# GeeeG/CloudAAE

Measured on AMD Instinct MI355X. Metric: point-clouds/sec (train step, N=1024), higher is better.
Workload: dtype f32, the dgcnn_agg products as error-free 3 x bf16 splits on the bf16 matrix cores (fp32 accumulate); 1 GPU; CloudAAE train step: get_model_dgcnn_mean_6d, all 21 YCB classes, batch 32/GPU, N=1024 points, k=10, 4N-point Chamfer target, TF-Adam; global_batch=32, per_gpu_batch=32, num_point=1024, parallelism=dp1, step_issue=recorded step replay

## Files before the change

cloudaae_amd/csrc/gemm_x3.hip:

```cpp
#include "common.h"
#include "gemm.h"
#include "bn_common.h"
#include "../../include/cloudaae_hip.h"

namespace cloudaae {

typedef float f32x16 __attribute__((ext_vector_type(16)));
typedef __bf16 bf16x8 __attribute__((ext_vector_type(8)));
typedef __bf16 bf16x2 __attribute__((ext_vector_type(2)));
typedef unsigned int u32x4v __attribute__((ext_vector_type(4)));

constexpr int X3_BK = 32;
constexpr int X3_LDK = 40;
constexpr int X3_THREADS = 256;

enum { X3_STORE = 0, X3_ACCUM = 1, X3_ATOMIC = 2 };

constexpr float X3_H_MAX = __builtin_bit_cast(float, 0x7f7f7fffu);
__device__ __forceinline__ void split3(float v, __bf16 &h, __bf16 &m, __bf16 &l)
{
    h = (__bf16)__builtin_amdgcn_fmed3f(v, -X3_H_MAX, X3_H_MAX);
    const float r1 = v - (float)h;
    m = (__bf16)r1;
    l = (__bf16)(r1 - (float)m);
}
__device__ __forceinline__ unsigned pack_pair(__bf16 lo, __bf16 hi)
{
    const bf16x2 p = {lo, hi};
    unsigned w;
    __builtin_memcpy(&w, &p, 4);
    return w;
}

template <int ROWS, bool KC>
struct Slab3 {
    static constexpr int ITEMS = KC ? ROWS * (X3_BK / 4) : (X3_BK / 2) * (ROWS / 4);
    static constexpr int PER = (ITEMS + X3_THREADS - 1) / X3_THREADS;
    static constexpr int PLANE = ROWS * X3_LDK;
    float4v r0[2][PER], r1[2][KC ? 1 : PER];
    unsigned boff[PER];
    static_assert(ROWS % 32 == 0, "tile sides are multiples of 32");
    static __device__ __forceinline__ int item_kp(int it) { return ((it >> 5) & 3) * 4 + (it & 3); }
    static __device__ __forceinline__ int item_oq(int it) { return (it >> 7) * 8 + ((it >> 2) & 7); }
    static __device__ __forceinline__ bool live(int it) { return ITEMS % X3_THREADS == 0 || it < ITEMS; }

    __device__ __forceinline__ void init(int ld)
    {
#pragma unroll
        for (int u = 0; u < PER; ++u) {
            const int it = u * X3_THREADS + (int)threadIdx.x;
            if (KC)
                boff[u] = 4u * (unsigned)((it / (X3_BK / 4)) * ld + 4 * (it % (X3_BK / 4)));
            else
                boff[u] = 4u * (unsigned)(2 * item_kp(it) * ld + 4 * item_oq(it));
        }
    }
    template <int SET>
    __device__ __forceinline__ void load(const float *__restrict__ P0, int ld)
    {
        const char *base = reinterpret_cast<const char *>(P0);
        const char *base1 = reinterpret_cast<const char *>(P0 + ld);
#pragma unroll
        for (int u = 0; u < PER; ++u) {
            const int it = u * X3_THREADS + (int)threadIdx.x;
            if (live(it)) {
                r0[SET][u] = *reinterpret_cast<const float4v *>(base + boff[u]);
                if (!KC)
                    r1[SET][u] = *reinterpret_cast<const float4v *>(base1 + boff[u]);
            }
        }
    }
    template <int SET>
    __device__ __forceinline__ void stage(__bf16 *__restrict__ lds) const
    {
#pragma unroll
        for (int u = 0; u < PER; ++u) {
            const int it = u * X3_THREADS + (int)threadIdx.x;
            if (!live(it))
                continue;
            __bf16 a[3][4];
            split3(r0[SET][u].x, a[0][0], a[1][0], a[2][0]);
            split3(r0[SET][u].y, a[0][1], a[1][1], a[2][1]);
            split3(r0[SET][u].z, a[0][2], a[1][2], a[2][2]);
            split3(r0[SET][u].w, a[0][3], a[1][3], a[2][3]);
            if (KC) {
                const int o = it / (X3_BK / 4), kq = it % (X3_BK / 4);
#pragma unroll
                for (int p = 0; p < 3; ++p) {
                    const unsigned w0 = pack_pair(a[p][0], a[p][1]), w1 = pack_pair(a[p][2], a[p][3]);
                    const uint2 w = {w0, w1};
                    *reinterpret_cast<uint2 *>(lds + p * PLANE + o * X3_LDK + 4 * kq) = w;
                }
            } else {
                __bf16 b[3][4];
                split3(r1[SET][u].x, b[0][0], b[1][0], b[2][0]);
                split3(r1[SET][u].y, b[0][1], b[1][1], b[2][1]);
                split3(r1[SET][u].z, b[0][2], b[1][2], b[2][2]);
                split3(r1[SET][u].w, b[0][3], b[1][3], b[2][3]);
                const int kp = item_kp(it), oq = item_oq(it);
                const int rot = (oq >> 1) & 3;
                const bool r1_ = (rot & 1) != 0, r2_ = (rot & 2) != 0;
#pragma unroll
                for (int p = 0; p < 3; ++p) {
                    const unsigned p0 = pack_pair(a[p][0], b[p][0]), p1 = pack_pair(a[p][1], b[p][1]),
                                   p2 = pack_pair(a[p][2], b[p][2]), p3 = pack_pair(a[p][3], b[p][3]);
                    const unsigned t0 = r1_ ? p1 : p0, t1 = r1_ ? p2 : p1, t2 = r1_ ? p3 : p2, t3 = r1_ ? p0 : p3;
                    const unsigned q0 = r2_ ? t2 : t0, q1 = r2_ ? t3 : t1, q2 = r2_ ? t0 : t2, q3 = r2_ ? t1 : t3;
                    __bf16 *dst = lds + p * PLANE + (4 * oq) * X3_LDK + 2 * kp;
                    *reinterpret_cast<unsigned *>(dst + ((0 + rot) & 3) * X3_LDK) = q0;
                    *reinterpret_cast<unsigned *>(dst + ((1 + rot) & 3) * X3_LDK) = q1;
                    *reinterpret_cast<unsigned *>(dst + ((2 + rot) & 3) * X3_LDK) = q2;
                    *reinterpret_cast<unsigned *>(dst + ((3 + rot) & 3) * X3_LDK) = q3;
                }
            }
        }
    }
};

template <int BM, int BN>
constexpr int x3_lds_bytes() { return 3 * (BM + BN) * X3_LDK * 2; }

template <int BM, int BN, int WM, int WN, bool TA, bool TB, int DEPTH>
__global__ __launch_bounds__(X3_THREADS, 2) void gemm_x3_kernel(int M, int N, int K, const float *__restrict__ A, int lda,
                                                             const float *__restrict__ B, int ldb, float *__restrict__ C,
                                                             int ldc, const float *__restrict__ bias, int epilogue,
                                                             int kchunk, double *__restrict__ colstats)
{
    static_assert(WM * WN * 64 == X3_THREADS, "4 waves");
    constexpr int TM = BM / WM / 32, TN = BN / WN / 32;
    typedef Slab3<BM, !TA> SA;
    typedef Slab3<BN, TB> SB;
    extern __shared__ __attribute__((aligned(16))) unsigned char x3_lds[];
    __bf16 *ldsA = reinterpret_cast<__bf16 *>(x3_lds);
    __bf16 *ldsB = ldsA + 3 * SA::PLANE;

    const int lane = threadIdx.x & 63, wave = threadIdx.x >> 6;
    const int wm = wave / WN, wn = wave % WN;
    const int tiles = gridDim.x * gridDim.y;
    int vid, slice;
    if (gridDim.z > 1 && (gridDim.z & 7) == 0) {
        const int lin = (blockIdx.z * gridDim.y + blockIdx.y) * gridDim.x + blockIdx.x;
        const int u = lin >> 3;
        slice = (lin & 7) + 8 * (u / tiles);
        vid = u % tiles;
    } else {
        vid = xcd_contiguous(blockIdx.y * gridDim.x + blockIdx.x, tiles);
        slice = blockIdx.z;
    }
    const int m0 = (vid / (int)gridDim.x) * BM, n0 = (vid % (int)gridDim.x) * BN;
    const int kbeg = slice * kchunk;
    const int kend = min(K, kbeg + kchunk);
    f32x16 acc[TM][TN];
#pragma unroll
    for (int i = 0; i < TM; ++i)
#pragma unroll
        for (int j = 0; j < TN; ++j)
#pragma unroll
            for (int r = 0; r < 16; ++r)
                acc[i][j][r] = 0.0f;

    const float *pa = A + (TA ? (size_t)kbeg * lda + m0 : (size_t)m0 * lda + kbeg);
    const float *pb = B + (TB ? (size_t)n0 * ldb + kbeg : (size_t)kbeg * ldb + n0);
    const size_t stepa = TA ? (size_t)X3_BK * lda : (size_t)X3_BK;
    const size_t stepb = TB ? (size_t)X3_BK : (size_t)X3_BK * ldb;
    SA sa;
    SB sb;
    sa.init(lda);
    sb.init(ldb);
    const int fr = lane & 31, fk = lane >> 5;
    auto multiply = [&]() {
#pragma unroll
        for (int s = 0; s < X3_BK / 16; ++s) {
            bf16x8 a[3][TM], b[3][TN];
#pragma unroll
            for (int p = 0; p < 3; ++p) {
#pragma unroll
                for (int i = 0; i < TM; ++i)
                    a[p][i] = *reinterpret_cast<const bf16x8 *>(ldsA + p * SA::PLANE + ((wm * TM + i) * 32 + fr) * X3_LDK +
                                                                16 * s + 8 * fk);
#pragma unroll
                for (int j = 0; j < TN; ++j)
                    b[p][j] = *reinterpret_cast<const bf16x8 *>(ldsB + p * SB::PLANE + ((wn * TN + j) * 32 + fr) * X3_LDK +
                                                                16 * s + 8 * fk);
            }
#pragma unroll
            for (int i = 0; i < TM; ++i)
#pragma unroll
                for (int j = 0; j < TN; ++j) {
                    acc[i][j] = __builtin_amdgcn_mfma_f32_32x32x16_bf16(a[2][i], b[0][j], acc[i][j], 0, 0, 0);
                    acc[i][j] = __builtin_amdgcn_mfma_f32_32x32x16_bf16(a[0][i], b[2][j], acc[i][j], 0, 0, 0);
                    acc[i][j] = __builtin_amdgcn_mfma_f32_32x32x16_bf16(a[1][i], b[1][j], acc[i][j], 0, 0, 0);
                    acc[i][j] = __builtin_amdgcn_mfma_f32_32x32x16_bf16(a[1][i], b[0][j], acc[i][j], 0, 0, 0);
                    acc[i][j] = __builtin_amdgcn_mfma_f32_32x32x16_bf16(a[0][i], b[1][j], acc[i][j], 0, 0, 0);
                    acc[i][j] = __builtin_amdgcn_mfma_f32_32x32x16_bf16(a[0][i], b[0][j], acc[i][j], 0, 0, 0);
                }
        }
    };
    if (DEPTH == 2) {
        const int nslab = (kend - kbeg) / X3_BK;
        auto slab_a = [&](int i) { return pa + (size_t)(i < nslab ? i : nslab - 1) * stepa; };
        auto slab_b = [&](int i) { return pb + (size_t)(i < nslab ? i : nslab - 1) * stepb; };
        sa.template load<0>(slab_a(0), lda);
        sb.template load<0>(slab_b(0), ldb);
        __builtin_amdgcn_sched_barrier(0);
        sa.template load<1>(slab_a(1), lda);
        sb.template load<1>(slab_b(1), ldb);
        __builtin_amdgcn_sched_barrier(0);
        for (int i = 0; i < nslab; i += 2) {
            __syncthreads();
            sa.template stage<0>(ldsA);
            sb.template stage<0>(ldsB);
            __syncthreads();
            sa.template load<0>(slab_a(i + 2), lda);
            sb.template load<0>(slab_b(i + 2), ldb);
            __builtin_amdgcn_sched_barrier(0);
            multiply();
            __builtin_amdgcn_sched_barrier(0);
            __syncthreads();
            sa.template stage<1>(ldsA);
            sb.template stage<1>(ldsB);
            __syncthreads();
            sa.template load<1>(slab_a(i + 3), lda);
            sb.template load<1>(slab_b(i + 3), ldb);
            __builtin_amdgcn_sched_barrier(0);
            multiply();
            __builtin_amdgcn_sched_barrier(0);
        }
    } else {
        sa.template load<0>(pa, lda);
        sb.template load<0>(pb, ldb);
        for (int k0 = kbeg; k0 < kend; k0 += X3_BK) {
            __syncthreads();
            sa.template stage<0>(ldsA);
            sb.template stage<0>(ldsB);
            __syncthreads();
            if (k0 + X3_BK < kend) {
                pa += stepa;
                pb += stepb;
                sa.template load<0>(pa, lda);
                sb.template load<0>(pb, ldb);
            }
            multiply();
        }
    }

    const bool add_bias = bias != nullptr && (epilogue != X3_ATOMIC || slice == 0);
    if (colstats != nullptr) {
        __syncthreads();
        double (*cs)[WM][BN] = reinterpret_cast<double (*)[WM][BN]>(x3_lds);
#pragma unroll
        for (int j = 0; j < TN; ++j) {
            const int cl = (wn * TN + j) * 32 + fr;
            const float bv = add_bias ? bias[n0 + cl] : 0.0f;
            double s1 = 0.0, s2 = 0.0;
#pragma unroll
            for (int i = 0; i < TM; ++i)
#pragma unroll
                for (int r = 0; r < 16; ++r) {
                    const double v = (double)(acc[i][j][r] + bv);
                    s1 += v;
                    s2 += v * v;
                }
            s1 += __shfl_xor(s1, 32, 64);
            s2 += __shfl_xor(s2, 32, 64);
            if (fk == 0) {
                cs[0][wm][cl] = s1;
                cs[1][wm][cl] = s2;
            }
        }
        __syncthreads();
        for (int t = threadIdx.x; t < 2 * BN; t += X3_THREADS) {
            const int which = t / BN, cl = t % BN;
            double v = cs[which][0][cl];
#pragma unroll
            for (int w = 1; w < WM; ++w)
                v += cs[which][w][cl];
            colstats[((size_t)(m0 / BM) * 2 + which) * N + n0 + cl] = v;
        }
    }
    float *c0 = C + (size_t)(m0 + wm * TM * 32 + 4 * fk) * ldc + (n0 + wn * TN * 32 + fr);
#pragma unroll
    for (int j = 0; j < TN; ++j) {
        const float bv = add_bias ? bias[n0 + (wn * TN + j) * 32 + fr] : 0.0f;
#pragma unroll
        for (int i = 0; i < TM; ++i) {
#pragma unroll
            for (int r = 0; r < 16; ++r) {
                float *dst = c0 + (size_t)(i * 32 + (r & 3) + 8 * (r >> 2)) * ldc + j * 32;
                const float v = acc[i][j][r] + bv;
                if (epilogue == X3_STORE)
                    *dst = v;
                else if (epilogue == X3_ACCUM)
                    *dst = *dst + v;
                else
                    atomicAdd(dst, v);
            }
        }
    }
}

static bool gemm_x3_plan(int ta, int tb, int M, int N, int K, int &BM, int &BN, int &splits)
{
    if (M <= 0 || N <= 0 || K <= 0 || K % X3_BK != 0 || (ta && tb))
        return false;
    BM = (ta && M % 160 == 0 && M % 128 != 0) ? 160 : 128;
    BN = (!ta && tb && N % 160 == 0 && N % 128 != 0) ? 160 : 128;
    if (M % BM != 0 || N % BN != 0)
        return false;
    const long long tiles = (long long)(M / BM) * (N / BN);
    splits = 1;
    if (tiles < 256 && K >= 256) {
        splits = (int)((tiles <= 4 ? 256 : 512) / tiles);
        const int max_splits = K / 128 > 0 ? K / 128 : 1;
        if (splits > max_splits)
            splits = max_splits;
        if (splits < 1)
            splits = 1;
        if (splits > 8)
            splits = splits / 8 * 8;
    }
    return true;
}

template <int BM, int BN, int WM, int WN, bool TA, bool TB, int DEPTH>
static int launch_x3(const char *name, dim3 grid, hipStream_t s, int M, int N, int K, const float *A, int lda, const float *B,
                     int ldb, float *C, int ldc, const float *bias, int epi, int kchunk, double *cs)
{
    constexpr int bytes = x3_lds_bytes<BM, BN>();
    constexpr auto kernel = &gemm_x3_kernel<BM, BN, WM, WN, TA, TB, DEPTH>;
    CLOUDAAE_CHECK_HIP(allow_dynamic_lds<kernel>(bytes, bytes), name);
    hipLaunchKernelGGL(kernel, grid, dim3(X3_THREADS), bytes, s, M, N, K, A, lda, B, ldb, C,
                       ldc, bias, epi, kchunk, cs);
    return 0;
}


__device__ __forceinline__ void split8(const float4v &x, const float4v &y, bf16x8 &h, bf16x8 &m, bf16x8 &l)
{
    const float v[8] = {x.x, x.y, x.z, x.w, y.x, y.y, y.z, y.w};
#pragma unroll
    for (int e = 0; e < 8; ++e) {
        const __bf16 hh = (__bf16)__builtin_amdgcn_fmed3f(v[e], -X3_H_MAX, X3_H_MAX);
        const float r1 = v[e] - (float)hh;
        const __bf16 mm = (__bf16)r1;
        h[e] = hh;
        m[e] = mm;
        l[e] = (__bf16)(r1 - (float)mm);
    }
}

__global__ __launch_bounds__(256) void x3_split_kernel(int rows0, int K0, int tr0, __bf16 *__restrict__ planes0, int rows1, int K1,
                                                       int tr1, __bf16 *__restrict__ planes1, const float *__restrict__ src, int ld)
{
    const bool second = blockIdx.y != 0;
    const int rows = second ? rows1 : rows0, K = second ? K1 : K0, transposed = second ? tr1 : tr0;
    __bf16 *__restrict__ planes = second ? planes1 : planes0;
    const int units = K >> 3;
    const long long t = (long long)blockIdx.x * 256 + threadIdx.x;
    if (t >= (long long)rows * units)
        return;
    int n, u;
    float4v x, y;
    if (transposed) {
        n = (int)(t % rows);
        u = (int)(t / rows);
        const float *s = src + (size_t)(8 * u) * ld + n;
        x = float4v{s[0], s[(size_t)ld], s[(size_t)2 * ld], s[(size_t)3 * ld]};
        y = float4v{s[(size_t)4 * ld], s[(size_t)5 * ld], s[(size_t)6 * ld], s[(size_t)7 * ld]};
    } else {
        u = (int)(t % units);
        n = (int)(t / units);
        const float4v *s = reinterpret_cast<const float4v *>(src + (size_t)n * ld + 8 * u);
        x = s[0];
        y = s[1];
    }
    bf16x8 h, m, l;
    split8(x, y, h, m, l);
    const int step = u >> 1, q = (u & 1) ^ ((n >> 3) & 1);
    __bf16 *d = planes + ((size_t)step * 3 * rows + n) * 16 + q * 8;
    *reinterpret_cast<bf16x8 *>(d) = h;
    *reinterpret_cast<bf16x8 *>(d + (size_t)rows * 16) = m;
    *reinterpret_cast<bf16x8 *>(d + (size_t)2 * rows * 16) = l;
}

template <int TM, int TN, int AS>
struct X3S {
    static constexpr int BM = 128 * TM, BN = 32 * TN;
    static constexpr int A_WAVE = 32 * TM * 128;
    static constexpr int A_STAGE = 4 * A_WAVE;
    static constexpr int A_BYTES = AS * A_STAGE;
    static constexpr int P_PLANE = BN * 32;
    static constexpr int P_STAGE = 3 * P_PLANE;
    static constexpr int P_PIECES = 3 * TN;
    static constexpr int LDS = A_BYTES + 3 * P_STAGE;
    static constexpr int JB = (TN - 1) / 2;
    static constexpr int T_STAGE = BN_DYC * 32 * 4;
    static constexpr int LDS_BNB = LDS + AS * T_STAGE;
};

struct X3BnBwd {
    const float *consts;
    float *dy;
    int lddy, rows, relu;
};

template <int TM, int TN, int AS, bool BNB>
__global__ __launch_bounds__(256, 2) void gemm_x3s_kernel(int M, int N, int K, const float *__restrict__ A, int lda,
                                                          const __bf16 *__restrict__ P, float *__restrict__ C, int ldc,
                                                          const float *__restrict__ bias, int accumulate,
                                                          double *__restrict__ colstats, X3BnBwd f)
{
    typedef X3S<TM, TN, AS> G;
    extern __shared__ __attribute__((aligned(16))) unsigned char x3_lds[];
    const int lane = threadIdx.x & 63;
    const int wave = __builtin_amdgcn_readfirstlane((int)(threadIdx.x >> 6));
    const int fr = lane & 31, fk = lane >> 5;
    const int tiles_n = N / G::BN;
    const int vid = xcd_contiguous(blockIdx.x, gridDim.x);
    const int m0 = (vid / tiles_n) * G::BM, n0 = (vid % tiles_n) * G::BN;
    const int nslab = K >> 5, nstep = K >> 4;

    const float *asrc = A + (size_t)(m0 + wave * 32 * TM + (lane >> 3)) * lda + 4 * ((lane & 7) ^ (lane >> 4));
    const size_t a8 = (size_t)8 * lda;
    unsigned char *lds_a = x3_lds + wave * G::A_WAVE;
    const float *tsrc = BNB ? f.consts + (size_t)(m0 / f.rows) * (size_t)(K >> 5) * (BN_DYC * 32) + wave * 64 + lane : nullptr;
    unsigned char *lds_t = x3_lds + G::LDS + wave * 256;
    auto dma_a = [&](int slab, int stage) {
        const float *ga = asrc + (size_t)slab * 32;
        unsigned char *la = lds_a + stage * G::A_STAGE;
#pragma unroll
        for (int t = 0; t < 4 * TM; ++t)
            __builtin_amdgcn_global_load_lds(ga + t * a8 + ((t & 1) ? ((lane & 4) ? -16 : 16) : 0), la + t * 1024, 16, 0, 0);
        if (BNB)
            __builtin_amdgcn_global_load_lds(tsrc + (size_t)slab * (BN_DYC * 32), lds_t + stage * G::T_STAGE, 4, 0, 0);
    };
    const int dybytes = (BNB && n0 == 0) ? (int)(((size_t)(G::BM - 1) * f.lddy + K) * sizeof(float)) : 0;
    const __amdgpu_buffer_rsrc_t dyrs = __builtin_amdgcn_make_buffer_rsrc(
        f.dy + (size_t)__builtin_amdgcn_readfirstlane(m0) * f.lddy, 0, __builtin_amdgcn_readfirstlane(dybytes), 0x00020000);
    const unsigned dyoff = (unsigned)((wave * 32 * TM + fr) * f.lddy + 8 * fk) * 4u;
    const bool relu = BNB && f.relu != 0;
    const __bf16 *psrc = P + (size_t)n0 * 16 + 8 * lane;
    const size_t pplane = (size_t)N * 16, pstep = 3 * pplane;
    auto dma_p = [&](int step, int ring) {
        unsigned char *sp = x3_lds + G::A_BYTES + ring * G::P_STAGE;
        const __bf16 *gp = psrc + (size_t)step * pstep;
#pragma unroll
        for (int i = 0; i < (G::P_PIECES + 3) / 4; ++i) {
            const int pc = wave + 4 * i;
            if (G::P_PIECES % 4 == 0 || pc < G::P_PIECES) {
                const int plane = pc / TN, rg = pc % TN;
                __builtin_amdgcn_global_load_lds(gp + plane * pplane + (size_t)rg * 512, sp + pc * 1024, 16, 0, 0);
            }
        }
    };

    const int swa = (fr >> 1) & 7;
    int offa[2][2];
#pragma unroll
    for (int ss = 0; ss < 2; ++ss)
#pragma unroll
        for (int hh = 0; hh < 2; ++hh)
            offa[ss][hh] = wave * G::A_WAVE + fr * 128 + (((4 * ss + 2 * fk + hh) ^ swa) << 4);
    const int offp = G::A_BYTES + fr * 32 + ((fk ^ ((fr >> 3) & 1)) << 4);

    f32x16 acc[TM][TN];
#pragma unroll
    for (int i = 0; i < TM; ++i)
#pragma unroll
        for (int j = 0; j < TN; ++j)
#pragma unroll
            for (int r = 0; r < 16; ++r)
                acc[i][j][r] = 0.0f;

    bf16x8 af[2][3][TM], bp[2][3];
    auto prepare_a = [&](int buf, int ss, int stage, int slab) {
        float4v cst[BN_DYC][2];
        if (BNB) {
#pragma unroll
            for (int q = 0; q < BN_DYC; ++q)
#pragma unroll
                for (int hh = 0; hh < 2; ++hh)
                    cst[q][hh] = *reinterpret_cast<const float4v *>(x3_lds + G::LDS + stage * G::T_STAGE + q * 128 +
                                                                    (16 * ss + 8 * fk + 4 * hh) * 4);
        }
#pragma unroll
        for (int i = 0; i < TM; ++i) {
            float4v x = *reinterpret_cast<const float4v *>(x3_lds + offa[ss][0] + i * 4096 + stage * G::A_STAGE);
            float4v y = *reinterpret_cast<const float4v *>(x3_lds + offa[ss][1] + i * 4096 + stage * G::A_STAGE);
            if (BNB) {
                float4v *v[2] = {&x, &y};
#pragma unroll
                for (int hh = 0; hh < 2; ++hh)
#pragma unroll
                    for (int e = 0; e < 4; ++e)
                        (*v[hh])[e] = bn_bwd_dy_hoisted((*v[hh])[e], cst[BN_DYC_SC][hh][e], cst[BN_DYC_SH][hh][e],
                                                        cst[BN_DYC_MEAN][hh][e], cst[BN_DYC_RSTD][hh][e], cst[BN_DYC_M2][hh][e],
                                                        cst[BN_DYC_GR][hh][e], cst[BN_DYC_A0][hh][e], cst[BN_DYC_A1][hh][e], relu);
                const unsigned o = dyoff + (unsigned)(i * 32 * f.lddy + slab * 32 + 16 * ss) * 4u;
                __builtin_amdgcn_raw_buffer_store_b128(__builtin_bit_cast(u32x4v, x), dyrs, o, 0, 0);
                __builtin_amdgcn_raw_buffer_store_b128(__builtin_bit_cast(u32x4v, y), dyrs, o + 16u, 0, 0);
            }
            split8(x, y, af[buf][0][i], af[buf][1][i], af[buf][2][i]);
        }
    };
    auto read_p = [&](int pb, int ring, int j) {
#pragma unroll
        for (int p = 0; p < 3; ++p)
            bp[pb][p] = *reinterpret_cast<const bf16x8 *>(x3_lds + offp + ring * G::P_STAGE + p * G::P_PLANE + j * 1024);
    };
    auto tile = [&](int abuf, int pb, int j) {
        constexpr int PA[6] = {2, 0, 1, 1, 0, 0}, PB[6] = {0, 2, 1, 0, 1, 0};
#pragma unroll
        for (int q = 0; q < 6; ++q)
#pragma unroll
            for (int i = 0; i < TM; ++i)
                acc[i][j] = __builtin_amdgcn_mfma_f32_32x32x16_bf16(af[abuf][PA[q]][i], bp[pb][PB[q]], acc[i][j], 0, 0, 0);
    };
    auto step = [&](int g, int ring, int abuf, int pb0, bool second_half) {
        const int ring1 = ring == 2 ? 0 : ring + 1, ring2 = ring == 0 ? 2 : ring - 1;
        const int slab = g >> 1, ast = AS == 2 ? (slab & 1) : 0;
        if (!second_half)
            prepare_a(abuf ^ 1, 1, ast, slab);
#pragma unroll
        for (int j = 0; j < TN; ++j) {
            const int pb = (pb0 + j) & 1;
            if (j + 1 < TN)
                read_p(pb ^ 1, ring, j + 1);
            else
                read_p(pb ^ 1, ring1, 0);
            tile(abuf, pb, j);
            if (j == G::JB) {
                if (AS == 2 && second_half)
                    asm volatile("s_waitcnt vmcnt(%0) lgkmcnt(0)" ::"n"(4 * TM + (BNB ? 1 : 0)) : "memory");
                else
                    asm volatile("s_waitcnt vmcnt(0) lgkmcnt(0)" ::: "memory");
                __builtin_amdgcn_s_barrier();
                asm volatile("" ::: "memory");
                dma_p(min(g + 2, nstep - 1), ring2);
                if (!second_half)
                    dma_a(min(slab + AS, nslab - 1), ast);
                else
                    prepare_a(abuf ^ 1, 0, AS == 2 ? (ast ^ 1) : 0, min(slab + 1, nslab - 1));
            }
        }
    };

    dma_a(0, 0);
    if (AS == 2)
        dma_a(min(1, nslab - 1), 1);
    dma_p(0, 0);
    asm volatile("s_waitcnt vmcnt(0)" ::: "memory");
    __syncthreads();
    dma_p(min(1, nstep - 1), 1);
    prepare_a(0, 0, 0, 0);
    read_p(0, 0, 0);
    int ring = 0;
    for (int s = 0; s < nslab; ++s) {
        step(2 * s, ring, 0, 0, false);
        ring = ring == 2 ? 0 : ring + 1;
        step(2 * s + 1, ring, 1, TN & 1, true);
        ring = ring == 2 ? 0 : ring + 1;
    }
    asm volatile("s_waitcnt vmcnt(0)" ::: "memory");
    __syncthreads();

    const int wrow = m0 + wave * 32 * TM;
    if (colstats != nullptr) {
        double (*cs)[4][G::BN] = reinterpret_cast<double (*)[4][G::BN]>(x3_lds);
#pragma unroll
        for (int j = 0; j < TN; ++j) {
            const int cl = j * 32 + fr;
            const float bv = bias != nullptr ? bias[n0 + cl] : 0.0f;
            double s1 = 0.0, s2 = 0.0;
#pragma unroll
            for (int i = 0; i < TM; ++i)
#pragma unroll
                for (int r = 0; r < 16; ++r) {
                    const double v = (double)(acc[i][j][r] + bv);
                    s1 += v;
                    s2 += v * v;
                }
            s1 += __shfl_xor(s1, 32, 64);
            s2 += __shfl_xor(s2, 32, 64);
            if (fk == 0) {
                cs[0][wave][cl] = s1;
                cs[1][wave][cl] = s2;
            }
        }
        __syncthreads();
        for (int t = threadIdx.x; t < 2 * G::BN; t += 256) {
            const int which = t / G::BN, cl = t % G::BN;
            const double v = ((cs[which][0][cl] + cs[which][1][cl]) + cs[which][2][cl]) + cs[which][3][cl];
            colstats[((size_t)(m0 / G::BM) * 2 + which) * N + n0 + cl] = v;
        }
    }
    float *c0 = C + (size_t)(wrow + 4 * fk) * ldc + (n0 + fr);
#pragma unroll
    for (int j = 0; j < TN; ++j) {
        const float bv = bias != nullptr ? bias[n0 + j * 32 + fr] : 0.0f;
#pragma unroll
        for (int i = 0; i < TM; ++i) {
#pragma unroll
            for (int r = 0; r < 16; ++r) {
                float *dst = c0 + (size_t)(i * 32 + (r & 3) + 8 * (r >> 2)) * ldc + j * 32;
                const float v = acc[i][j][r] + bv;
                *dst = accumulate ? *dst + v : v;
            }
        }
    }
}

template <int TM, int TN, int AS, bool BNB = false>
static int launch_x3s(const char *name, hipStream_t s, int M, int N, int K, const float *A, int lda, const void *planes, float *C,
                      int ldc, const float *bias, int accumulate, double *cs, X3BnBwd f = X3BnBwd{nullptr, nullptr, 0, 1, 0})
{
    typedef X3S<TM, TN, AS> G;
    constexpr int bytes = BNB ? G::LDS_BNB : G::LDS;
    static_assert(bytes <= 80 * 1024, "two workgroups per CU");
    constexpr auto kernel = &gemm_x3s_kernel<TM, TN, AS, BNB>;
    CLOUDAAE_CHECK_HIP(allow_dynamic_lds<kernel>(bytes, bytes), name);
    const int tiles = (M / G::BM) * (N / G::BN);
    hipLaunchKernelGGL(kernel, dim3(tiles), dim3(256), bytes, s, M, N, K, A, lda,
                       reinterpret_cast<const __bf16 *>(planes), C, ldc, bias, accumulate, cs, f);
    return 0;
}

static bool gemm_x3s_plan(int M, int N, int K, int &TM, int &TN)
{
    if (M <= 0 || N <= 0 || K <= 0 || K % 32 != 0 || M % 128 != 0)
        return false;
    TN = N % 128 == 0 ? 4 : (N % 160 == 0 ? 5 : 0);
    if (TN == 0)
        return false;
    TM = (TN == 4 && M % 256 == 0 && (long long)(M / 256) * (N / 128) >= 512) ? 2 : 1;
    return true;
}

bool gemm_x3s_bnbwd_served(int M, int N, int K, int rows)
{
    int TM, TN;
    return gemm_x3s_plan(M, N, K, TM, TN) && TM == 1 && TN == 5 && rows > 0 && rows % 128 == 0 && M % rows == 0;
}

int gemm_x3s_bnbwd_launch(const char *name, int M, int N, int K, const float *y, int ldy, const void *planes, float *dx, int lddx,
                          const float *consts, int rows, int relu, float *dy, int lddy, hipStream_t stream)
{
    CLOUDAAE_REQUIRE(gemm_x3s_bnbwd_served(M, N, K, rows), name, "product not served");
    CLOUDAAE_REQUIRE(ldy >= K && lddy >= K && lddx >= N && ldy % 4 == 0 && lddy % 4 == 0, name, "bad leading dimension");
    const int rc = launch_x3s<1, 5, 2, true>(name, stream, M, N, K, y, ldy, planes, dx, lddx, nullptr, 0, nullptr,
                                             X3BnBwd{consts, dy, lddy, rows, relu});
    if (rc != 0)
        return rc;
    CLOUDAAE_CHECK_LAUNCH(name);
    return 0;
}

}

using namespace cloudaae;

CLOUDAAE_API long long cloudaae_x3_planes_bytes(int rows, int k)
{
    return rows > 0 && k > 0 && k % 32 == 0 ? (long long)rows * k * 6 : 0;
}

CLOUDAAE_API int cloudaae_x3_split(int rows, int k, const float *src, int ld, int transposed, void *planes, cloudaae_stream_t stream)
{
    const char *name = "cloudaae_x3_split";
    CLOUDAAE_REQUIRE(rows > 0 && k > 0 && k % 32 == 0 && src && planes, name, "rows, k > 0, k a multiple of 32, non-null pointers");
    CLOUDAAE_REQUIRE(ld >= (transposed ? rows : k), name, "leading dimension too small");
    CLOUDAAE_REQUIRE(transposed || (ld % 4 == 0 && ((uintptr_t)src & 15) == 0), name, "rows must be 16-byte aligned");
    CLOUDAAE_REQUIRE(((uintptr_t)planes & 15) == 0, name, "planes must be 16-byte aligned");
    const long long items = (long long)rows * (k / 8);
    hipLaunchKernelGGL(x3_split_kernel, dim3((unsigned)((items + 255) / 256), 1), dim3(256), 0, (hipStream_t)stream, rows, k, transposed,
                       reinterpret_cast<__bf16 *>(planes), 0, 0, 0, (__bf16 *)nullptr, src, ld);
    CLOUDAAE_CHECK_LAUNCH(name);
    return 0;
}

CLOUDAAE_API int cloudaae_x3_split_weight(int K, int N, const float *W, int ldw, void *planes_fwd, void *planes_bwd,
                                          cloudaae_stream_t stream)
{
    const char *name = "cloudaae_x3_split_weight";
    CLOUDAAE_REQUIRE(K > 0 && N > 0 && K % 32 == 0 && N % 32 == 0 && W && planes_fwd && planes_bwd, name,
                     "K, N multiples of 32, non-null pointers");
    CLOUDAAE_REQUIRE(ldw >= N && ldw % 4 == 0 && ((uintptr_t)W & 15) == 0, name, "rows of W must be 16-byte aligned");
    CLOUDAAE_REQUIRE(((uintptr_t)planes_fwd & 15) == 0 && ((uintptr_t)planes_bwd & 15) == 0, name, "planes must be 16-byte aligned");
    const long long items = (long long)K * N / 8;
    hipLaunchKernelGGL(x3_split_kernel, dim3((unsigned)((items + 255) / 256), 2), dim3(256), 0, (hipStream_t)stream, N, K, 1,
                       reinterpret_cast<__bf16 *>(planes_fwd), K, N, 0, reinterpret_cast<__bf16 *>(planes_bwd), W, ldw);
    CLOUDAAE_CHECK_LAUNCH(name);
    return 0;
}

CLOUDAAE_API int cloudaae_gemm_bf16x3p_supported(int M, int N, int K)
{
    int TM, TN;
    return gemm_x3s_plan(M, N, K, TM, TN) ? 1 : 0;
}

CLOUDAAE_API int cloudaae_gemm_bf16x3p_colstats_parts(int M, int N, int K)
{
    int TM, TN;
    return gemm_x3s_plan(M, N, K, TM, TN) ? M / (128 * TM) : 0;
}

CLOUDAAE_API int cloudaae_gemm_bf16x3p(int M, int N, int K, const float *A, int lda, const void *planes, float *C, int ldc,
                                       const float *bias, int accumulate, double *colstats, cloudaae_stream_t stream)
{
    const char *name = "cloudaae_gemm_bf16x3p";
    int TM, TN;
    CLOUDAAE_REQUIRE(gemm_x3s_plan(M, N, K, TM, TN), name,
                     "product not served (M % 128 == 0, N a multiple of 128 or 160, K % 32 == 0; see cloudaae_gemm_bf16x3p_supported)");
    CLOUDAAE_REQUIRE(A && planes && C, name, "null argument");
    CLOUDAAE_REQUIRE(lda >= K && ldc >= N, name, "leading dimension too small");
    CLOUDAAE_REQUIRE(lda % 4 == 0 && ((uintptr_t)A & 15) == 0 && ((uintptr_t)planes & 15) == 0, name,
                     "operand rows must be 16-byte aligned");
    CLOUDAAE_REQUIRE(colstats == nullptr || accumulate == 0, name, "column statistics need an overwriting product");
    hipStream_t s = (hipStream_t)stream;
    int rc;
    if (TM == 2)
        rc = launch_x3s<2, 4, 1>(name, s, M, N, K, A, lda, planes, C, ldc, bias, accumulate, colstats);
    else if (TN == 4)
        rc = launch_x3s<1, 4, 2>(name, s, M, N, K, A, lda, planes, C, ldc, bias, accumulate, colstats);
    else
        rc = launch_x3s<1, 5, 2>(name, s, M, N, K, A, lda, planes, C, ldc, bias, accumulate, colstats);
    if (rc != 0)
        return rc;
    CLOUDAAE_CHECK_LAUNCH(name);
    return 0;
}

CLOUDAAE_API int cloudaae_gemm_bf16x3_supported(int trans_a, int trans_b, int M, int N, int K)
{
    int BM, BN, splits;
    return gemm_x3_plan(trans_a, trans_b, M, N, K, BM, BN, splits) ? 1 : 0;
}

CLOUDAAE_API int cloudaae_gemm_bf16x3_colstats_parts(int M, int N, int K)
{
    int BM, BN, splits;
    if (!gemm_x3_plan(0, 0, M, N, K, BM, BN, splits) || splits != 1)
        return 0;
    int TMs, TNs;
    if (gemm_x3s_plan(M, N, K, TMs, TNs) &&
        (long long)(M / (128 * TMs)) * (N / (32 * TNs)) >= 192)
        return M / (128 * TMs);
    return M / BM;
}

CLOUDAAE_API int cloudaae_gemm_bf16x3(int trans_a, int trans_b, int M, int N, int K, const float *A, int lda, const float *B,
                                      int ldb, float *C, int ldc, const float *bias, int accumulate, double *colstats,
                                      cloudaae_stream_t stream)
{
    const char *name = "cloudaae_gemm_bf16x3";
    int BM, BN, splits;
    CLOUDAAE_REQUIRE(gemm_x3_plan(trans_a, trans_b, M, N, K, BM, BN, splits), name,
                     "product not served (whole tiles of 128 / 160 and K a multiple of 32; see cloudaae_gemm_bf16x3_supported)");
    CLOUDAAE_REQUIRE(A && B && C, name, "null argument");
    CLOUDAAE_REQUIRE(lda >= (trans_a ? M : K) && ldb >= (trans_b ? K : N) && ldc >= N, name, "leading dimension too small");
    CLOUDAAE_REQUIRE(lda % 4 == 0 && ldb % 4 == 0 && ((uintptr_t)A & 15) == 0 && ((uintptr_t)B & 15) == 0, name,
                     "operand rows must be 16-byte aligned");
    hipStream_t s = (hipStream_t)stream;
    int TMs, TNs;
    if (!trans_a && gemm_x3s_plan(M, N, K, TMs, TNs) && (long long)(M / (128 * TMs)) * (N / (32 * TNs)) >= 192) {
        void *planes = nullptr;
        CLOUDAAE_CHECK_HIP(scratch_alloc(&planes, (size_t)cloudaae_x3_planes_bytes(N, K), s), name);
        int rc = cloudaae_x3_split(N, K, B, ldb, trans_b ? 0 : 1, planes, stream);
        if (rc == 0)
            rc = cloudaae_gemm_bf16x3p(M, N, K, A, lda, planes, C, ldc, bias, accumulate, colstats, stream);
        CLOUDAAE_CHECK_HIP(hipFreeAsync(planes, s), name);
        return rc;
    }
    int kchunk = ceil_div(ceil_div(K, splits), X3_BK) * X3_BK;
    splits = ceil_div(K, kchunk);
    CLOUDAAE_REQUIRE(colstats == nullptr || (splits == 1 && accumulate == 0), name,
                     "column statistics need an unsplit, overwriting product");
    int epi = accumulate == 1 ? X3_ACCUM : X3_STORE;
    if (splits > 1) {
        epi = X3_ATOMIC;
        if (!accumulate)
            CLOUDAAE_CHECK_HIP(hipMemset2DAsync(C, sizeof(float) * (size_t)ldc, 0, sizeof(float) * (size_t)N, (size_t)M, s),
                               name);
    }
    CLOUDAAE_REQUIRE(M / BM <= 65535, name, "M too large");
    dim3 grid(N / BN, M / BM, splits);
    int rc;
    if (!trans_a && !trans_b)
        rc = launch_x3<128, 128, 2, 2, false, false, 1>(name, grid, s, M, N, K, A, lda, B, ldb, C, ldc, bias, epi, kchunk, colstats);
    else if (!trans_a && BN == 160)
        rc = launch_x3<128, 160, 4, 1, false, true, 1>(name, grid, s, M, N, K, A, lda, B, ldb, C, ldc, bias, epi, kchunk, colstats);
    else if (!trans_a)
        rc = launch_x3<128, 128, 2, 2, false, true, 1>(name, grid, s, M, N, K, A, lda, B, ldb, C, ldc, bias, epi, kchunk, colstats);
    else if (BM == 160)
        rc = launch_x3<160, 128, 1, 4, true, false, 1>(name, grid, s, M, N, K, A, lda, B, ldb, C, ldc, bias, epi, kchunk, colstats);
    else
        rc = launch_x3<128, 128, 2, 2, true, false, 1>(name, grid, s, M, N, K, A, lda, B, ldb, C, ldc, bias, epi, kchunk, colstats);
    if (rc != 0)
        return rc;
    CLOUDAAE_CHECK_LAUNCH(name);
    return 0;
}
```

Measured before the change: 22080 clouds/s.

## Add software-pipelined weight-gradient x3 GEMM kernel for the 160x128 transposed-A path

Adds a dedicated kernel for the transposed-A 160x128 weight-gradient products that double-buffers LDS and register prefetches. It interleaves the bf16 three-way split and LDS staging of the next k-step with the MFMA work of the current one, using scheduling group barriers. LDS is sized to allow two workgroups per CU, and shared split helpers move to a header. It is on by default behind an env knob. It adds a large hand-scheduled kernel with swizzled layouts that carries correctness and register-pressure risk.

Result: no change. 22210 clouds/s (median of 6 runs) (+0.6%).

```diff
diff --git a/cloudaae_amd/csrc/gemm_x3.h b/cloudaae_amd/csrc/gemm_x3.h
--- /dev/null
+++ b/cloudaae_amd/csrc/gemm_x3.h
@@ -0,0 +1,36 @@
+#pragma once
+#include <hip/hip_runtime.h>
+#include "common.h"
+
+namespace cloudaae {
+
+typedef float f32x16 __attribute__((ext_vector_type(16)));
+typedef __bf16 bf16x8 __attribute__((ext_vector_type(8)));
+typedef __bf16 bf16x2 __attribute__((ext_vector_type(2)));
+typedef unsigned int u32x4v __attribute__((ext_vector_type(4)));
+
+constexpr int X3_BK = 32;
+constexpr int X3_THREADS = 256;
+
+enum { X3_STORE = 0, X3_ACCUM = 1, X3_ATOMIC = 2 };
+
+constexpr float X3_H_MAX = __builtin_bit_cast(float, 0x7f7f7fffu);
+__device__ __forceinline__ void split3(float v, __bf16 &h, __bf16 &m, __bf16 &l)
+{
+    h = (__bf16)__builtin_amdgcn_fmed3f(v, -X3_H_MAX, X3_H_MAX);
+    const float r1 = v - (float)h;
+    m = (__bf16)r1;
+    l = (__bf16)(r1 - (float)m);
+}
+__device__ __forceinline__ unsigned pack_pair(__bf16 lo, __bf16 hi)
+{
+    const bf16x2 p = {lo, hi};
+    unsigned w;
+    __builtin_memcpy(&w, &p, 4);
+    return w;
+}
+
+int gemm_x3dw_launch(const char *name, dim3 grid, hipStream_t s, int M, int N, int K, const float *A, int lda, const float *B,
+                     int ldb, float *C, int ldc, const float *bias, int epilogue, int kchunk, double *colstats);
+
+}
diff --git a/cloudaae_amd/csrc/gemm_x3.hip b/cloudaae_amd/csrc/gemm_x3.hip
--- a/cloudaae_amd/csrc/gemm_x3.hip
+++ b/cloudaae_amd/csrc/gemm_x3.hip
@@ -1,36 +1,12 @@
 #include "common.h"
 #include "gemm.h"
+#include "gemm_x3.h"
 #include "bn_common.h"
 #include "../../include/cloudaae_hip.h"
 
 namespace cloudaae {
 
-typedef float f32x16 __attribute__((ext_vector_type(16)));
-typedef __bf16 bf16x8 __attribute__((ext_vector_type(8)));
-typedef __bf16 bf16x2 __attribute__((ext_vector_type(2)));
-typedef unsigned int u32x4v __attribute__((ext_vector_type(4)));
-
-constexpr int X3_BK = 32;
 constexpr int X3_LDK = 40;
-constexpr int X3_THREADS = 256;
-
-enum { X3_STORE = 0, X3_ACCUM = 1, X3_ATOMIC = 2 };
-
-constexpr float X3_H_MAX = __builtin_bit_cast(float, 0x7f7f7fffu);
-__device__ __forceinline__ void split3(float v, __bf16 &h, __bf16 &m, __bf16 &l)
-{
-    h = (__bf16)__builtin_amdgcn_fmed3f(v, -X3_H_MAX, X3_H_MAX);
-    const float r1 = v - (float)h;
-    m = (__bf16)r1;
-    l = (__bf16)(r1 - (float)m);
-}
-__device__ __forceinline__ unsigned pack_pair(__bf16 lo, __bf16 hi)
-{
-    const bf16x2 p = {lo, hi};
-    unsigned w;
-    __builtin_memcpy(&w, &p, 4);
-    return w;
-}
 
 template <int ROWS, bool KC>
 struct Slab3 {
@@ -792,6 +768,8 @@
         rc = launch_x3<128, 160, 4, 1, false, true, 1>(name, grid, s, M, N, K, A, lda, B, ldb, C, ldc, bias, epi, kchunk, colstats);
     else if (!trans_a)
         rc = launch_x3<128, 128, 2, 2, false, true, 1>(name, grid, s, M, N, K, A, lda, B, ldb, C, ldc, bias, epi, kchunk, colstats);
+    else if (BM == 160 && CLOUDAAE_KNOB("CLOUDAAE_X3_DW_PIPELINED", 1) != 0)
+        rc = gemm_x3dw_launch(name, grid, s, M, N, K, A, lda, B, ldb, C, ldc, bias, epi, kchunk, colstats);
     else if (BM == 160)
         rc = launch_x3<160, 128, 1, 4, true, false, 1>(name, grid, s, M, N, K, A, lda, B, ldb, C, ldc, bias, epi, kchunk, colstats);
     else
diff --git a/cloudaae_amd/csrc/gemm_x3_dw.hip b/cloudaae_amd/csrc/gemm_x3_dw.hip
--- /dev/null
+++ b/cloudaae_amd/csrc/gemm_x3_dw.hip
@@ -0,0 +1,234 @@
+#include "common.h"
+#include "gemm_x3.h"
+#include "../../include/cloudaae_hip.h"
+
+namespace cloudaae {
+
+namespace {
+
+constexpr int DW_BM = 160, DW_BN = 128, DW_TM = 5;
+constexpr int DW_A_PLANE = DW_BM * 32, DW_B_PLANE = DW_BN * 32;
+constexpr int DW_B_BASE = 3 * DW_A_PLANE;
+constexpr int DW_BUF = 3 * (DW_A_PLANE + DW_B_PLANE);
+constexpr int DW_LDS = 2 * DW_BUF;
+static_assert(DW_LDS <= 80 * 1024, "two workgroups per CU");
+
+__device__ __forceinline__ int dw_row(int fr)
+{
+    const int q = fr >> 2, e = fr & 3;
+    return 16 * (q >> 2) + 8 * (e >> 1) + 4 * (e & 1) + ((q & 3) ^ e);
+}
+
+struct DwRegs {
+    float4v a0, a1, b0, b1;
+    float d0, d1;
+};
+
+}
+
+__global__ __launch_bounds__(X3_THREADS, 2) void gemm_x3dw_kernel(int M, int N, int K, const float *__restrict__ A, int lda,
+                                                                const float *__restrict__ B, int ldb, float *__restrict__ C,
+                                                                int ldc, const float *__restrict__ bias, int epilogue,
+                                                                int kchunk, double *__restrict__ colstats)
+{
+    extern __shared__ __attribute__((aligned(16))) unsigned char x3_lds[];
+    const int tid = threadIdx.x;
+    const int lane = tid & 63, wave = __builtin_amdgcn_readfirstlane(tid >> 6);
+    const int fr = lane & 31, fk = lane >> 5;
+    const int tiles = gridDim.x * gridDim.y;
+    int vid, slice;
+    if (gridDim.z > 1 && (gridDim.z & 7) == 0) {
+        const int lin = (blockIdx.z * gridDim.y + blockIdx.y) * gridDim.x + blockIdx.x;
+        const int u = lin >> 3;
+        slice = (lin & 7) + 8 * (u / tiles);
+        vid = u % tiles;
+    } else {
+        vid = xcd_contiguous(blockIdx.y * gridDim.x + blockIdx.x, tiles);
+        slice = blockIdx.z;
+    }
+    const int m0 = (vid / (int)gridDim.x) * DW_BM, n0 = (vid % (int)gridDim.x) * DW_BN;
+    const int kbeg = slice * kchunk;
+    const int kend = min(K, kbeg + kchunk);
+    const int nstep = (kend - kbeg) >> 4;
+
+    const int l32 = tid & 31, h8 = tid >> 5;
+    const int kp = l32 >> 2, oq = 4 * h8 + (l32 & 3);
+    const int kpd = 4 * (h8 & 1) + (l32 >> 3), frd = 8 * (h8 >> 1) + (l32 & 7);
+    const float *ga = A + (size_t)(kbeg + 2 * kp) * lda + m0 + 4 * oq;
+    const float *gb = B + (size_t)(kbeg + 2 * kp) * ldb + n0 + 4 * oq;
+    const float *gd = A + (size_t)(kbeg + 2 * kpd) * lda + m0 + 128 + frd;
+    const size_t stepa = (size_t)16 * lda, stepb = (size_t)16 * ldb;
+    const int q2 = (oq >> 2) & 1;
+    const int wbase = (32 * (oq >> 3) + 16 * q2) * 32 + (((kp >> 2) ^ q2) << 4) + 4 * (kp & 3);
+    int woff[4];
+#pragma unroll
+    for (int e = 0; e < 4; ++e)
+        woff[e] = wbase + (8 * (e >> 1) + 4 * (e & 1) + ((oq & 3) ^ e)) * 32;
+    const int woffd = (128 + dw_row(frd)) * 32 + (((kpd >> 2) ^ (frd >> 4)) << 4) + 4 * (kpd & 3);
+    const int roff = dw_row(fr) * 32 + ((fk ^ (fr >> 4)) << 4);
+    const int roffb = DW_B_BASE + wave * 1024 + roff;
+
+    auto load = [&](DwRegs &r, int step) {
+        const int s = step < nstep ? step : nstep - 1;
+        const float *pa = ga + (size_t)s * stepa, *pb = gb + (size_t)s * stepb, *pd = gd + (size_t)s * stepa;
+        r.a0 = *reinterpret_cast<const float4v *>(pa);
+        r.a1 = *reinterpret_cast<const float4v *>(pa + lda);
+        r.b0 = *reinterpret_cast<const float4v *>(pb);
+        r.b1 = *reinterpret_cast<const float4v *>(pb + ldb);
+        r.d0 = pd[0];
+        r.d1 = pd[lda];
+    };
+    auto put = [&](float v0, float v1, unsigned char *dst, int plane) {
+        __bf16 x[3], y[3];
+        split3(v0, x[0], x[1], x[2]);
+        split3(v1, y[0], y[1], y[2]);
+#pragma unroll
+        for (int p = 0; p < 3; ++p)
+            *reinterpret_cast<unsigned *>(dst + p * plane) = pack_pair(x[p], y[p]);
+    };
+    auto stage = [&](const DwRegs &r, int buf, int part) {
+        unsigned char *la = x3_lds + buf * DW_BUF, *lb = la + DW_B_BASE;
+        if (part == 0) {
+            put(r.a0.x, r.a1.x, la + woff[0], DW_A_PLANE);
+            put(r.a0.y, r.a1.y, la + woff[1], DW_A_PLANE);
+            put(r.d0, r.d1, la + woffd, DW_A_PLANE);
+        } else if (part == 1) {
+            put(r.a0.z, r.a1.z, la + woff[2], DW_A_PLANE);
+            put(r.a0.w, r.a1.w, la + woff[3], DW_A_PLANE);
+        } else if (part == 2) {
+            put(r.b0.x, r.b1.x, lb + woff[0], DW_B_PLANE);
+            put(r.b0.y, r.b1.y, lb + woff[1], DW_B_PLANE);
+        } else {
+            put(r.b0.z, r.b1.z, lb + woff[2], DW_B_PLANE);
+            put(r.b0.w, r.b1.w, lb + woff[3], DW_B_PLANE);
+        }
+    };
+
+    f32x16 acc[DW_TM];
+#pragma unroll
+    for (int i = 0; i < DW_TM; ++i)
+#pragma unroll
+        for (int r = 0; r < 16; ++r)
+            acc[i][r] = 0.0f;
+    bf16x8 af[2][3], bf[2][3];
+    auto read_a = [&](int set, int buf, int i) {
+#pragma unroll
+        for (int p = 0; p < 3; ++p)
+            af[set][p] = *reinterpret_cast<const bf16x8 *>(x3_lds + buf * DW_BUF + p * DW_A_PLANE + i * 1024 + roff);
+    };
+    auto read_b = [&](int set, int buf) {
+#pragma unroll
+        for (int p = 0; p < 3; ++p)
+            bf[set][p] = *reinterpret_cast<const bf16x8 *>(x3_lds + buf * DW_BUF + p * DW_B_PLANE + roffb);
+    };
+    auto tile = [&](int aset, int bset, int i) {
+        constexpr int PA[6] = {2, 0, 1, 1, 0, 0}, PB[6] = {0, 2, 1, 0, 1, 0};
+#pragma unroll
+        for (int q = 0; q < 6; ++q)
+            acc[i] = __builtin_amdgcn_mfma_f32_32x32x16_bf16(af[aset][PA[q]], bf[bset][PB[q]], acc[i], 0, 0, 0);
+    };
+
+    DwRegs regs[2];
+    auto step = [&](int s, int par) {
+#pragma unroll
+        for (int i = 0; i < DW_TM; ++i) {
+            const int aset = (par + i) & 1;
+            if (i < DW_TM - 1) {
+                read_a(aset ^ 1, par, i + 1);
+                stage(regs[par ^ 1], par ^ 1, i);
+            } else {
+                load(regs[par ^ 1], s + 3);
+                __syncthreads();
+                read_a(aset ^ 1, par ^ 1, 0);
+                read_b(par ^ 1, par ^ 1);
+            }
+            tile(aset, par, i);
+            if (i < DW_TM - 1) {
+                __builtin_amdgcn_sched_group_barrier(0x100, 3, 0);
+#pragma unroll
+                for (int q = 0; q < 6; ++q) {
+                    __builtin_amdgcn_sched_group_barrier(0x008, 1, 0);
+                    __builtin_amdgcn_sched_group_barrier(0x002, 7, 0);
+                    __builtin_amdgcn_sched_group_barrier(0x200, 2, 0);
+                }
+            }
+            __builtin_amdgcn_sched_barrier(0);
+        }
+    };
+
+    load(regs[0], 0);
+    __builtin_amdgcn_sched_barrier(0);
+    load(regs[1], 1);
+    __builtin_amdgcn_sched_barrier(0);
+#pragma unroll
+    for (int part = 0; part < 4; ++part)
+        stage(regs[0], 0, part);
+    load(regs[0], 2);
+    __syncthreads();
+    read_a(0, 0, 0);
+    read_b(0, 0);
+    __builtin_amdgcn_sched_barrier(0);
+    for (int s = 0; s < nstep; s += 2) {
+        step(s, 0);
+        step(s + 1, 1);
+    }
+
+    const bool add_bias = bias != nullptr && (epilogue != X3_ATOMIC || slice == 0);
+    if (colstats != nullptr) {
+        __syncthreads();
+        double (*cs)[DW_BN] = reinterpret_cast<double (*)[DW_BN]>(x3_lds);
+        const int cl = wave * 32 + fr;
+        const float bv = add_bias ? bias[n0 + cl] : 0.0f;
+        double s1 = 0.0, s2 = 0.0;
+#pragma unroll
+        for (int i = 0; i < DW_TM; ++i)
+#pragma unroll
+            for (int r = 0; r < 16; ++r) {
+                const double v = (double)(acc[i][r] + bv);
+                s1 += v;
+                s2 += v * v;
+            }
+        s1 += __shfl_xor(s1, 32, 64);
+        s2 += __shfl_xor(s2, 32, 64);
+        if (fk == 0) {
+            cs[0][cl] = s1;
+            cs[1][cl] = s2;
+        }
+        __syncthreads();
+        for (int t = tid; t < 2 * DW_BN; t += X3_THREADS) {
+            const int which = t / DW_BN, c = t % DW_BN;
+            colstats[((size_t)(m0 / DW_BM) * 2 + which) * N + n0 + c] = cs[which][c];
+        }
+    }
+    float *c0 = C + (size_t)(m0 + 4 * fk) * ldc + (n0 + wave * 32 + fr);
+    const float bv = add_bias ? bias[n0 + wave * 32 + fr] : 0.0f;
+#pragma unroll
+    for (int i = 0; i < DW_TM; ++i) {
+#pragma unroll
+        for (int r = 0; r < 16; ++r) {
+            float *dst = c0 + (size_t)(i * 32 + (r & 3) + 8 * (r >> 2)) * ldc;
+            const float v = acc[i][r] + bv;
+            if (epilogue == X3_STORE)
+                *dst = v;
+            else if (epilogue == X3_ACCUM)
+                *dst = *dst + v;
+            else
+                atomicAdd(dst, v);
+        }
+    }
+}
+
+int gemm_x3dw_launch(const char *name, dim3 grid, hipStream_t s, int M, int N, int K, const float *A, int lda, const float *B,
+                     int ldb, float *C, int ldc, const float *bias, int epilogue, int kchunk, double *colstats)
+{
+    CLOUDAAE_REQUIRE(M % DW_BM == 0 && N % DW_BN == 0 && K % X3_BK == 0 && kchunk % X3_BK == 0 && (int)grid.x == N / DW_BN &&
+                         (int)grid.y == M / DW_BM,
+                     name, "product not served by the pipelined weight-gradient kernel");
+    constexpr auto kernel = &gemm_x3dw_kernel;
+    CLOUDAAE_CHECK_HIP(allow_dynamic_lds<kernel>(DW_LDS, DW_LDS), name);
+    hipLaunchKernelGGL(kernel, grid, dim3(X3_THREADS), DW_LDS, s, M, N, K, A, lda, B, ldb, C, ldc, bias, epilogue, kchunk,
+                       colstats);
+    return 0;
+}
+
+}
```
